# AlwinEsch/pvr.rtl.radiofm

Hardware: AMD Instinct MI355X
Metric: IQ MS/s demodulated (whole node) + achieved HBM GB/s on FIR stage (higher is better)
Workload: dtype f32

## Files before the change

pvr.rtl.radiofm_amd/csrc/fmd_batch.hip:

```cpp
#include "../../include/fmd.h"

#include <hip/hip_runtime.h>
#include <hip/hip_ext.h>

#include <algorithm>
#include <chrono>
#include <cmath>
#include <cstdio>
#include <cstdlib>
#include <cstring>
#include <deque>
#include <functional>
#include <map>
#include <memory>
#include <mutex>
#include <string>
#include <utility>
#include <vector>

#include "fmd_design.hpp"
#include "fmd_groups.hpp"
#include "fmd_kernels.hip.h"
#include "fmd_receiver.hpp"

// ... 603 lines not shown
      push(0, 0, 0);
    const size_t g = steps.size();
    for (size_t i = f; i < g; i++)
    {
      const int far = steps[std::min(i + size_t(fmd::HBF_NSET - 1), g - 1)].a_lo - steps[i].a_lo;
      if (far < 0 || far > 63 || g - i > 1023)
        return nullptr;
      steps[i].n |= unsigned(far) << fmd::HBF_FAR_SHIFT;
      if (steps[i].n & (fmd::HBF_TAIL0 | fmd::HBF_TAIL1))
        steps[i].n |= unsigned(g - i) << fmd::HBF_TAILS_SHIFT;
    }
    steps[g - 1].n |= fmd::HBF_LAST;
    fmd::HbStep hdr[2];
    static_assert(sizeof(hdr) == sizeof(tails), "HbTails in the place of two records");
    std::memcpy(hdr, &tails, sizeof(tails));
    steps.push_back(hdr[0]);
    steps.push_back(hdr[1]);
  }
  first.push_back(int(steps.size()));
  std::unique_ptr<fmd_batch::HbfPlan> pl(new fmd_batch::HbfPlan);
  pl->n_in = n_in;
  pl->S = unsigned(first.size() - 1);
  if (pl->steps.alloc(steps.size()) || pl->seg_first.alloc(first.size()) ||
      upload(pl->steps.p, steps.data(), steps.size() * sizeof(fmd::HbStep)) ||
      upload(pl->seg_first.p, first.data(), first.size() * sizeof(int)))
    return nullptr;
  if (b->hbf_plans.size() >= 16)
  {
    (void)hipDeviceSynchronize();
    b->hbf_plans.erase(b->hbf_plans.begin());
  }
  b->hbf_plans.push_back(std::move(pl));
  return b->hbf_plans.back().get();
}

bool rsr_configure(fmd_batch* b, int form)
{
  static const int forms[3][2] = {{2, 8}, {4, 4}, {2, 4}};
  const fmd::Design& d = b->des;
  const int R = forms[form][0], NW = forms[form][1];
  const double step = double(d.rs_step);
  const unsigned per_step = unsigned(NW * R);
  const unsigned span = d.rs_order + 1u + unsigned(std::ceil((per_step - 1) * step)) + 1u;
  const unsigned nbr = (span - 1u + 7u) / 8u + 2u;
  const unsigned new_rows = unsigned(std::ceil(per_step * step)) + 8u;
  b->rsr_R = 0;
  if (nbr > 39u || new_rows > unsigned(fmd::RSR_ROWS))
    return false;
  b->rsr_R = R;
  b->rsr_NW = NW;
  b->rsr_nbr = nbr;
  b->rsr_rb = int((d.rs_order + 7u) / 8u * 8u + 8u);
  const unsigned gspan = d.rs_order + 1u + unsigned(std::ceil((R - 1) * step)) + 1u;
  b->rsr_nbm = (gspan - 1u + 7u) / 8u + 2u + 1u;
  return true;
}

}

extern "C" {

const char* fmd_last_error(void)
{
  return g_err.c_str();
}

const char* fmd_version(void)
{
  return "fmd-hip 0.1 (gfx950)";
}

const char* fmd_stage_name(unsigned idx)
{
  return idx < ST_COUNT ? kStageNames[idx] : "";
}

}

namespace
{

int create_streams(fmd_batch* b)
{
  int lo = 0, hi = 0;
  HIPCHK(hipDeviceGetStreamPriorityRange(&lo, &hi));
  const int nstreams = 5;
  const int prio[5] = {hi, hi, lo, lo, lo};
  hipStream_t st4[5] = {nullptr, nullptr, nullptr, nullptr, nullptr};
  if (pick_independent_streams(nstreams, prio, st4, &b->streams_sharing) != 0)
    return fail(FMD_ERR_DEVICE, "could not create the internal streams");
  b->s_fir = st4[0];
  b->s_ser = st4[1];
  b->s_post = st4[2];
  b->s_rds = st4[3];
  b->s_lpf = st4[4];
  return FMD_OK;
}

int create_one(const fmd_params* params, unsigned n_channels, const int* tuning_shifts, int device,
               const fmd_callbacks* cb, void* user, fmd_batch* shell, fmd_batch** out)
{
  std::unique_ptr<fmd_batch> b(new fmd_batch);
  b->device = device;
  b->cparams = *params;
  b->params.sample_rate_if = params->sample_rate_if;
  b->params.tuning_offset = params->tuning_offset;
  b->params.sample_rate_pcm = params->sample_rate_pcm;
// ... 2163 lines not shown
```

pvr.rtl.radiofm_amd/csrc/fmd_k_resample.hip.h:

```cpp
#pragma once

#include "fmd_k_common.hip.h"

namespace fmd
{

__global__ void k_rs_table(const float* __restrict__ coeff, unsigned order, float p, float pstep,
                           unsigned A, float* __restrict__ ktab, unsigned row_stride, unsigned margin,
                           int* __restrict__ pidx)
{
  const unsigned i = blockIdx.x;
  if (i >= A)
    return;
  const float pf = p + (float)i * pstep;
  const int pi = (int)pf;
  const float k1 = pf - (float)pi;
  const float k0 = 1 - k1;
  for (unsigned j = threadIdx.x; j <= order; j += blockDim.x)
    ktab[(size_t)i * row_stride + margin + j] = coeff[j] * k0 + coeff[j + 1] * k1;
  if (threadIdx.x == 0)
    pidx[i] = pi;
}

#ifndef FMD_RS_R
// ... 74 lines not shown
    {
      bool fin = true;
#pragma unroll
      for (int q = 0; q < RS_B; q++)
        fin = fin && __builtin_isfinite(xs[q].x) && __builtin_isfinite(xs[q].y);
      literal = FMD_ANY_LANE(!fin);
    }
    if (!literal)
    {
#pragma unroll
      for (int q = 0; q < RS_B; q++)
      {
#pragma unroll
        for (int r = 0; r < RS_R; r++)
        {
          acc[r].x += kk[r][q] * xs[q].x;
          acc[r].y += kk[r][q] * xs[q].y;
        }
      }
    }
    else
    {
#pragma unroll
      for (int q = 0; q < RS_B; q++)
      {
#pragma unroll
        for (int r = 0; r < RS_R; r++)
        {
          const int j = t + q - off[r];
          if (j >= 0 && j <= (int)order)
          {
            acc[r].x += kk[r][q] * xs[q].x;
            acc[r].y += kk[r][q] * xs[q].y;
          }
        }
      }
    }
  }
  if (c < C)
  {
#pragma unroll
    for (int r = 0; r < RS_R; r++)
      if (r < nr)
        out[(size_t)(Hout + i0 + r) * CP + c] = make_float2(acc[r].y, acc[r].x);
  }
}


constexpr int RSR_ROWS = 96;
constexpr int RSR_HEAD = 4 + 4;

template <int R, bool FMA = false>
__device__ __forceinline__ void rs_walk_asm(fmd_f2v (&acc)[R], unsigned& off, unsigned& cnt, unsigned lane16,
                                            unsigned wrap, unsigned klo, unsigned khi, unsigned kinc);
template <>
__device__ __forceinline__ void rs_walk_asm<4, false>(fmd_f2v (&acc)[4], unsigned& off, unsigned& cnt,
                                                      unsigned lane16, unsigned wrap, unsigned klo, unsigned khi,
                                                      unsigned kinc)
{
#include "fmd_rs_walk_r4.inc"
}
template <>
__device__ __forceinline__ void rs_walk_asm<2, false>(fmd_f2v (&acc)[2], unsigned& off, unsigned& cnt,
                                                      unsigned lane16, unsigned wrap, unsigned klo, unsigned khi,
                                                      unsigned kinc)
{
#include "fmd_rs_walk_r2.inc"
}
template <>
__device__ __forceinline__ void rs_walk_asm<2, true>(fmd_f2v (&acc)[2], unsigned& off, unsigned& cnt,
                                                     unsigned lane16, unsigned wrap, unsigned klo, unsigned khi,
                                                     unsigned kinc)
{
#include "fmd_rs_walk_r2_fma.inc"
}

template <int R, int NW>
__device__ __forceinline__ void rs_warm_asm(unsigned tlo, unsigned thi, unsigned gstride, unsigned rounds,
                                            unsigned pace);
template <>
__device__ __forceinline__ void rs_warm_asm<4, 4>(unsigned tlo, unsigned thi, unsigned gstride, unsigned rounds,
                                                  unsigned pace)
{
#include "fmd_rs_warm_r4w4.inc"
}
template <>
__device__ __forceinline__ void rs_warm_asm<2, 8>(unsigned tlo, unsigned thi, unsigned gstride, unsigned rounds,
                                                  unsigned pace)
{
#include "fmd_rs_warm_r2w8.inc"
}
template <>
__device__ __forceinline__ void rs_warm_asm<2, 4>(unsigned tlo, unsigned thi, unsigned gstride, unsigned rounds,
                                                  unsigned pace)
{
#include "fmd_rs_warm_r2w4.inc"
}

template <int R, int RSR_NW>
__global__ __launch_bounds__(64) void k_rs_plan(const float* __restrict__ coeff, unsigned order, float p,
                                                float pstep, unsigned A, int RB, unsigned NBR,
                                                float* __restrict__ tab, unsigned nbm,
                                                int* __restrict__ head, int* __restrict__ steptab)
{
  const unsigned g = blockIdx.x;
  auto pidx_of = [&](unsigned i) { return (int)(p + (float)i * pstep); };
  auto extent = [&](unsigned gg, int& top, int& nb) {
    const unsigned i0 = gg * R;
    if (i0 >= A)
    {
      top = 0;
      nb = 0;
      return;
    }
    const unsigned il = min(i0 + R - 1, A - 1);
    top = (pidx_of(il) + RB) >> 3;
    const int bot = (pidx_of(i0) - (int)order + RB) >> 3;
    nb = top - bot + 1;
    nb += nb & 1;
  };
  int top, nb;
  extent(g, top, nb);
  float k0[R], k1[R];
  int pi[R];
#pragma unroll
  for (int r = 0; r < R; r++)
  {
    const unsigned i = min(g * R + r, A - 1);
    const float pf = p + (float)i * pstep;
    pi[r] = (int)pf;
    k1[r] = pf - (float)pi[r];
    k0[r] = 1 - k1[r];
  }
  for (int idx = threadIdx.x; idx < nb * 8 * R; idx += 64)
  {
    const int b = idx / (8 * R), q = (idx / R) & 7, r = idx % R;
    const int row = (top - b) * 8 + 7 - q - RB;
    float v = 0.0f;
#pragma unroll
    for (int rr = 0; rr < R; rr++)
      if (rr == r)
      {
        const int j = pi[rr] - row;
        if (j >= 0 && j <= (int)order)
          v = coeff[j] * k0[rr] + coeff[j + 1] * k1[rr];
      }
    tab[((size_t)g * nbm + b) * (8 * R) + (idx % (8 * R))] = v;
  }
  if (threadIdx.x == 0)
  {
    int* h = head + (size_t)g * RSR_HEAD;
    h[0] = top;
    h[1] = nb;
    h[2] = (int)(((unsigned)top % NBR) * 4096u);
    h[3] = 0;
#pragma unroll
    for (int r = 0; r < R; r++)
      h[4 + r] = pi[r];
    if (g % RSR_NW == 0)
    {
      int stop = 0, sbot = 0x7fffffff;
      for (unsigned w = 0; w < (unsigned)RSR_NW; w++)
      {
        int t, n;
        extent(g + w, t, n);
        if (n > 0)
        {
          stop = t;
          sbot = min(sbot, t - n + 1);
        }
      }
      steptab[2 * (g / RSR_NW)] = stop;
      steptab[2 * (g / RSR_NW) + 1] = sbot;
    }
  }
}

template <int R, int RSR_NW, bool FMA = false>
__global__ __launch_bounds__(64 * (RSR_NW + 1)) void k_resample_ring(
    const float2* __restrict__ br, unsigned Hbb, int RB, unsigned order, const float* __restrict__ tab,
    unsigned nbm, const int* __restrict__ head, const int* __restrict__ steptab, unsigned nsteps,
    unsigned steps_per_wg, unsigned NBR, unsigned A, float2* __restrict__ out, unsigned Hout, unsigned C,
    unsigned CP, unsigned prio)
{
  constexpr int RSR_PRE = RSR_ROWS / RSR_NW;
  constexpr int LEAD = 3;
  extern __shared__ __align__(16) unsigned char rsr_smem[];
  __shared__ unsigned nonfinite_s;
  const unsigned lane = threadIdx.x;
  const unsigned w = (unsigned)__builtin_amdgcn_readfirstlane((int)threadIdx.y);
  wave_prio(prio);
  const unsigned units = (CP / 64u) * nsteps;
  unsigned u0 = min(units, blockIdx.x * steps_per_wg);
  const unsigned u1 = min(units, u0 + steps_per_wg);
  if (u0 >= u1)
    return;
  unsigned c = 0, s0 = 0, s1 = 0, lane_off = 0;
  bool live = false;
  const unsigned ring_pairs = NBR * 4;
  const char* const gbase = reinterpret_cast<const char*>(br + ((ptrdiff_t)Hbb - (ptrdiff_t)RB) * (ptrdiff_t)CP);
  const size_t row_bytes = (size_t)CP * sizeof(float2);
  unsigned emax = 0u;
  auto look = [&](float2 v) {
    emax = max(emax, max(__float_as_uint(v.x) & 0x7fffffffu, __float_as_uint(v.y) & 0x7fffffffu));
  };
  auto ring_addr = [&](unsigned pair_slot, unsigned odd) {
    return reinterpret_cast<float2*>(rsr_smem + (size_t)pair_slot * 1024 + lane * 16 + odd * 8);
  };
  float2 pre[RSR_PRE];
  auto fetch = [&](int r0, int mine) {
    const char* rp = gbase + (size_t)(r0 + (int)w) * row_bytes;
#pragma unroll
    for (int n = 0; n < RSR_PRE; n++)
      if (n < mine)
      {
        const fmd_f2v v = __builtin_nontemporal_load(reinterpret_cast<const fmd_f2v*>(rp + lane_off));
        pre[n] = make_float2(v.x, v.y);
        rp += RSR_NW * row_bytes;
      }
  };
  auto stash = [&](int r0, int mine) {
    unsigned ps = ((unsigned)(r0 + (int)w) >> 1) % ring_pairs;
#pragma unroll
    for (int n = 0; n < RSR_PRE; n++)
      if (n < mine)
      {
        look(pre[n]);
        *ring_addr(ps, w & 1u) = pre[n];
        ps += RSR_NW / 2;
        ps = ps >= ring_pairs ? ps - ring_pairs : ps;
      }
    if (emax >= 0x7f800000u && live)
      nonfinite_s = 1u;
  };
  auto share = [&](int n_rows) { return (n_rows - (int)w + RSR_NW - 1) / RSR_NW; };
  const bool warmer = w == (unsigned)RSR_NW;
  auto warm = [&](unsigned step, int b0, int rounds) {
    if (rounds <= 0)
      return;
    const uint64_t ta = reinterpret_cast<uint64_t>(tab) + ((uint64_t)step * RSR_NW * nbm + (uint64_t)b0) * (32 * R);
    rs_warm_asm<R, RSR_NW>((unsigned)ta, (unsigned)(ta >> 32), nbm * (32u * R), (unsigned)rounds, 0u);
  };
  {
    const size_t gsz = (size_t)nbm * (8 * R) * sizeof(float);
    const char* t0 = reinterpret_cast<const char*>(tab);
    const size_t bytes = (size_t)nsteps * RSR_NW * gsz;
    const unsigned nx = (gridDim.x + 7u) / 8u, part = blockIdx.x / 8u;
    const size_t per = ((bytes + nx - 1) / nx + 15) & ~(size_t)15;
    const size_t lo = min(bytes, part * per), hi = min(bytes, lo + per);
    unsigned sink = 0;
    for (size_t o = lo + (size_t)(threadIdx.y * 64 + lane) * 16; o + 16 <= hi; o += (size_t)(RSR_NW + 1) * 64 * 16)
    {
      const uint4 v = *reinterpret_cast<const uint4*>(t0 + o);
      sink |= v.x ^ v.y ^ v.z ^ v.w;
    }
    if (sink == 0x7fc12345u)
      nonfinite_s = sink;
  }
  for (; u0 < u1; u0 += s1 - s0)
  {
  const unsigned grp = u0 / nsteps;
  s0 = u0 - grp * nsteps;
  s1 = min(nsteps, s0 + (u1 - u0));
  c = grp * 64 + lane;
  lane_off = c * (unsigned)sizeof(float2);
  live = c < C;
  emax = 0u;
  __syncthreads();
  if (threadIdx.x == 0 && threadIdx.y == 0)
    nonfinite_s = 0u;
  __syncthreads();
  int topb = steptab[2 * s0];
  {
    const int r_hi = topb * 8 + 7;
    for (int r0 = steptab[2 * s0 + 1] * 8; r0 <= r_hi; r0 += RSR_NW * RSR_PRE)
    {
      const int mine = warmer ? 0 : share(min(r_hi + 1 - r0, RSR_NW * RSR_PRE));
      fetch(r0, mine);
      stash(r0, mine);
    }
    if (warmer)
      warm(s0, 0, LEAD);
  }
  __syncthreads();
  for (unsigned s = s0; s < s1; s++)
  {
    const int ntop = s + 1 < s1 ? steptab[2 * (s + 1)] : topb;
    const int r_new0 = topb * 8 + 8;
    const int mine = warmer ? 0 : share((ntop - topb) * 8);
    fetch(r_new0, mine);
    if (warmer)
    {
      warm(s, LEAD, (int)nbm - 1 - LEAD);
      if (s + 1 < s1)
        warm(s + 1, 0, LEAD);
      lds_barrier();
      topb = ntop;
      lds_barrier();
      continue;
    }
    const unsigned g = s * RSR_NW + w;
    const int* __restrict__ h = head + (size_t)g * RSR_HEAD;
    const int gtop = h[0], nb = h[1];
    fmd_f2v acc[R];
#pragma unroll
    for (int r = 0; r < R; r++)
      acc[r] = fmd_f2v{0.0f, 0.0f};
    if (nb > 0)
    {
      const float* __restrict__ kp = tab + (size_t)g * nbm * (8 * R);
      if (__builtin_expect(nonfinite_s == 0u, 1))
      {
        unsigned off = (unsigned)h[2], cnt = (unsigned)nb >> 1;
        const uint64_t ka = reinterpret_cast<uint64_t>(kp);
        rs_walk_asm<R, FMA>(acc, off, cnt, (unsigned)(size_t)rsr_smem + lane * 16u, (NBR - 1u) * 4096u, (unsigned)ka,
                       (unsigned)(ka >> 32), 32u * R);
      }
      else
      {
        for (int b = 0; b < nb; b++)
        {
          const unsigned slot = (unsigned)(gtop - b) % NBR;
#pragma unroll
          for (int q = 0; q < 8; q++)
          {
            const int rowb = 7 - q;
            const float2 x = *ring_addr(slot * 4 + (unsigned)(rowb >> 1), (unsigned)rowb & 1u);
            const int row = (gtop - b) * 8 + rowb - RB;
#pragma unroll
            for (int r = 0; r < R; r++)
            {
              const int j = h[4 + r] - row;
              if (j >= 0 && j <= (int)order)
              {
                const float k = kp[(size_t)b * (8 * R) + q * R + r];
                if (FMA)
                {
                  acc[r].x = __builtin_fmaf(k, x.x, acc[r].x);
                  acc[r].y = __builtin_fmaf(k, x.y, acc[r].y);
                }
                else
                {
                  acc[r].x += k * x.x;
                  acc[r].y += k * x.y;
                }
              }
            }
          }
        }
      }
      if (live)
      {
#pragma unroll
        for (int r = 0; r < R; r++)
          if (g * R + r < A)
            out[(size_t)(Hout + g * R + r) * CP + c] = make_float2(acc[r].y, acc[r].x);
      }
    }
    lds_barrier();
    stash(r_new0, mine);
    topb = ntop;
    lds_barrier();
  }
  }
}

}
```

pvr.rtl.radiofm_amd/csrc/fmd_rs_walk_r2.inc:

```
asm volatile(
    "s_mov_b32 s34, %6\n\t"
    "s_mov_b32 s35, %7\n\t"
    "v_add_u32 v104, %2, %4\n\t"
    "s_load_dwordx16 s[36:51], s[34:35], 0x0\n\t"
    "ds_read_b128 v[76:79], v104 offset:3072\n\t"
    "ds_read_b128 v[72:75], v104 offset:2048\n\t"
    "ds_read_b128 v[68:71], v104 offset:1024\n\t"
    "ds_read_b128 v[64:67], v104\n\t"
    "s_add_u32 s34, s34, %8\n\t"
    "s_addc_u32 s35, s35, 0\n\t"
    "s_sub_u32 %2, %2, 4096\n\t"
    "s_cselect_b32 %2, %5, %2\n\t"
    "1:\n\t"
    "s_waitcnt lgkmcnt(0)\n\t"
    "v_add_u32 v104, %2, %4\n\t"
    "s_load_dwordx16 s[52:67], s[34:35], 0x0\n\t"
    "ds_read_b128 v[92:95], v104 offset:3072\n\t"
    "ds_read_b128 v[88:91], v104 offset:2048\n\t"
    "ds_read_b128 v[84:87], v104 offset:1024\n\t"
    "ds_read_b128 v[80:83], v104\n\t"
    "s_add_u32 s34, s34, %8\n\t"
    "s_addc_u32 s35, s35, 0\n\t"
    "s_sub_u32 %2, %2, 4096\n\t"
    "s_cselect_b32 %2, %5, %2\n\t"
    "v_pk_mul_f32 v[96:97], v[78:79], s[36:37] op_sel_hi:[1,0]\n\t"
    "v_pk_mul_f32 v[98:99], v[78:79], s[36:37] op_sel:[0,1]\n\t"
    "v_pk_add_f32 %0, %0, v[96:97]\n\t"
    "v_pk_mul_f32 v[100:101], v[76:77], s[38:39] op_sel_hi:[1,0]\n\t"
    "v_pk_add_f32 %1, %1, v[98:99]\n\t"
    "v_pk_mul_f32 v[102:103], v[76:77], s[38:39] op_sel:[0,1]\n\t"
    "v_pk_add_f32 %0, %0, v[100:101]\n\t"
    "v_pk_mul_f32 v[96:97], v[74:75], s[40:41] op_sel_hi:[1,0]\n\t"
    "v_pk_add_f32 %1, %1, v[102:103]\n\t"
    "v_pk_mul_f32 v[98:99], v[74:75], s[40:41] op_sel:[0,1]\n\t"
    "v_pk_add_f32 %0, %0, v[96:97]\n\t"
    "v_pk_mul_f32 v[100:101], v[72:73], s[42:43] op_sel_hi:[1,0]\n\t"
    "v_pk_add_f32 %1, %1, v[98:99]\n\t"
    "v_pk_mul_f32 v[102:103], v[72:73], s[42:43] op_sel:[0,1]\n\t"
    "v_pk_add_f32 %0, %0, v[100:101]\n\t"
    "v_pk_mul_f32 v[96:97], v[70:71], s[44:45] op_sel_hi:[1,0]\n\t"
    "v_pk_add_f32 %1, %1, v[102:103]\n\t"
    "v_pk_mul_f32 v[98:99], v[70:71], s[44:45] op_sel:[0,1]\n\t"
    "v_pk_add_f32 %0, %0, v[96:97]\n\t"
    "v_pk_mul_f32 v[100:101], v[68:69], s[46:47] op_sel_hi:[1,0]\n\t"
    "v_pk_add_f32 %1, %1, v[98:99]\n\t"
    "v_pk_mul_f32 v[102:103], v[68:69], s[46:47] op_sel:[0,1]\n\t"
    "v_pk_add_f32 %0, %0, v[100:101]\n\t"
    "v_pk_mul_f32 v[96:97], v[66:67], s[48:49] op_sel_hi:[1,0]\n\t"
    "v_pk_add_f32 %1, %1, v[102:103]\n\t"
    "v_pk_mul_f32 v[98:99], v[66:67], s[48:49] op_sel:[0,1]\n\t"
    "v_pk_add_f32 %0, %0, v[96:97]\n\t"
    "v_pk_mul_f32 v[100:101], v[64:65], s[50:51] op_sel_hi:[1,0]\n\t"
    "v_pk_add_f32 %1, %1, v[98:99]\n\t"
    "v_pk_mul_f32 v[102:103], v[64:65], s[50:51] op_sel:[0,1]\n\t"
    "v_pk_add_f32 %0, %0, v[100:101]\n\t"
    "v_pk_add_f32 %1, %1, v[102:103]\n\t"
    "s_waitcnt lgkmcnt(0)\n\t"
    "v_add_u32 v104, %2, %4\n\t"
    "s_load_dwordx16 s[36:51], s[34:35], 0x0\n\t"
    "ds_read_b128 v[76:79], v104 offset:3072\n\t"
    "ds_read_b128 v[72:75], v104 offset:2048\n\t"
    "ds_read_b128 v[68:71], v104 offset:1024\n\t"
    "ds_read_b128 v[64:67], v104\n\t"
    "s_add_u32 s34, s34, %8\n\t"
    "s_addc_u32 s35, s35, 0\n\t"
    "s_sub_u32 %2, %2, 4096\n\t"
    "s_cselect_b32 %2, %5, %2\n\t"
    "v_pk_mul_f32 v[96:97], v[94:95], s[52:53] op_sel_hi:[1,0]\n\t"
    "v_pk_mul_f32 v[98:99], v[94:95], s[52:53] op_sel:[0,1]\n\t"
    "v_pk_add_f32 %0, %0, v[96:97]\n\t"
    "v_pk_mul_f32 v[100:101], v[92:93], s[54:55] op_sel_hi:[1,0]\n\t"
    "v_pk_add_f32 %1, %1, v[98:99]\n\t"
    "v_pk_mul_f32 v[102:103], v[92:93], s[54:55] op_sel:[0,1]\n\t"
    "v_pk_add_f32 %0, %0, v[100:101]\n\t"
    "v_pk_mul_f32 v[96:97], v[90:91], s[56:57] op_sel_hi:[1,0]\n\t"
    "v_pk_add_f32 %1, %1, v[102:103]\n\t"
    "v_pk_mul_f32 v[98:99], v[90:91], s[56:57] op_sel:[0,1]\n\t"
    "v_pk_add_f32 %0, %0, v[96:97]\n\t"
    "v_pk_mul_f32 v[100:101], v[88:89], s[58:59] op_sel_hi:[1,0]\n\t"
    "v_pk_add_f32 %1, %1, v[98:99]\n\t"
    "v_pk_mul_f32 v[102:103], v[88:89], s[58:59] op_sel:[0,1]\n\t"
    "v_pk_add_f32 %0, %0, v[100:101]\n\t"
    "v_pk_mul_f32 v[96:97], v[86:87], s[60:61] op_sel_hi:[1,0]\n\t"
    "v_pk_add_f32 %1, %1, v[102:103]\n\t"
    "v_pk_mul_f32 v[98:99], v[86:87], s[60:61] op_sel:[0,1]\n\t"
    "v_pk_add_f32 %0, %0, v[96:97]\n\t"
    "v_pk_mul_f32 v[100:101], v[84:85], s[62:63] op_sel_hi:[1,0]\n\t"
    "v_pk_add_f32 %1, %1, v[98:99]\n\t"
    "v_pk_mul_f32 v[102:103], v[84:85], s[62:63] op_sel:[0,1]\n\t"
    "v_pk_add_f32 %0, %0, v[100:101]\n\t"
    "v_pk_mul_f32 v[96:97], v[82:83], s[64:65] op_sel_hi:[1,0]\n\t"
    "v_pk_add_f32 %1, %1, v[102:103]\n\t"
    "v_pk_mul_f32 v[98:99], v[82:83], s[64:65] op_sel:[0,1]\n\t"
    "v_pk_add_f32 %0, %0, v[96:97]\n\t"
    "v_pk_mul_f32 v[100:101], v[80:81], s[66:67] op_sel_hi:[1,0]\n\t"
    "v_pk_add_f32 %1, %1, v[98:99]\n\t"
    "v_pk_mul_f32 v[102:103], v[80:81], s[66:67] op_sel:[0,1]\n\t"
    "v_pk_add_f32 %0, %0, v[100:101]\n\t"
    "v_pk_add_f32 %1, %1, v[102:103]\n\t"
    "s_sub_u32 %3, %3, 1\n\t"
    "s_cmp_lg_u32 %3, 0\n\t"
    "s_cbranch_scc1 1b\n\t"
    "s_waitcnt lgkmcnt(0)\n\t"
    : "+v"(acc[0]), "+v"(acc[1]), "+s"(off), "+s"(cnt)
    : "v"(lane16), "s"(wrap), "s"(klo), "s"(khi), "s"(kinc)
    : "v64", "v65", "v66", "v67", "v68", "v69", "v70", "v71", "v72", "v73", "v74", "v75", "v76",
      "v77", "v78", "v79", "v80", "v81", "v82", "v83", "v84", "v85", "v86", "v87", "v88", "v89",
      "v90", "v91", "v92", "v93", "v94", "v95", "v96", "v97", "v98", "v99", "v100", "v101", "v102",
      "v103", "v104", "s34", "s35", "s36", "s37", "s38", "s39", "s40", "s41", "s42", "s43", "s44",
      "s45", "s46", "s47", "s48", "s49", "s50", "s51", "s52", "s53", "s54", "s55", "s56", "s57",
      "s58", "s59", "s60", "s61", "s62", "s63", "s64", "s65", "s66", "s67", "scc", "memory");
```

pvr.rtl.radiofm_amd/csrc/fmd_rs_walk_r2_fma.inc:

```
asm volatile(
    "s_mov_b32 s34, %6\n\t"
    "s_mov_b32 s35, %7\n\t"
    "v_add_u32 v104, %2, %4\n\t"
    "s_load_dwordx16 s[36:51], s[34:35], 0x0\n\t"
    "ds_read_b128 v[76:79], v104 offset:3072\n\t"
    "ds_read_b128 v[72:75], v104 offset:2048\n\t"
    "ds_read_b128 v[68:71], v104 offset:1024\n\t"
    "ds_read_b128 v[64:67], v104\n\t"
    "s_add_u32 s34, s34, %8\n\t"
    "s_addc_u32 s35, s35, 0\n\t"
    "s_sub_u32 %2, %2, 4096\n\t"
    "s_cselect_b32 %2, %5, %2\n\t"
    "1:\n\t"
    "s_waitcnt lgkmcnt(0)\n\t"
    "v_add_u32 v104, %2, %4\n\t"
    "s_load_dwordx16 s[52:67], s[34:35], 0x0\n\t"
    "ds_read_b128 v[92:95], v104 offset:3072\n\t"
    "ds_read_b128 v[88:91], v104 offset:2048\n\t"
    "ds_read_b128 v[84:87], v104 offset:1024\n\t"
    "ds_read_b128 v[80:83], v104\n\t"
    "s_add_u32 s34, s34, %8\n\t"
    "s_addc_u32 s35, s35, 0\n\t"
    "s_sub_u32 %2, %2, 4096\n\t"
    "s_cselect_b32 %2, %5, %2\n\t"
    "v_pk_fma_f32 %0, v[78:79], s[36:37], %0 op_sel_hi:[1,0,1]\n\t"
    "v_pk_fma_f32 %1, v[78:79], s[36:37], %1 op_sel:[0,1,0]\n\t"
    "v_pk_fma_f32 %0, v[76:77], s[38:39], %0 op_sel_hi:[1,0,1]\n\t"
    "v_pk_fma_f32 %1, v[76:77], s[38:39], %1 op_sel:[0,1,0]\n\t"
    "v_pk_fma_f32 %0, v[74:75], s[40:41], %0 op_sel_hi:[1,0,1]\n\t"
    "v_pk_fma_f32 %1, v[74:75], s[40:41], %1 op_sel:[0,1,0]\n\t"
    "v_pk_fma_f32 %0, v[72:73], s[42:43], %0 op_sel_hi:[1,0,1]\n\t"
    "v_pk_fma_f32 %1, v[72:73], s[42:43], %1 op_sel:[0,1,0]\n\t"
    "v_pk_fma_f32 %0, v[70:71], s[44:45], %0 op_sel_hi:[1,0,1]\n\t"
    "v_pk_fma_f32 %1, v[70:71], s[44:45], %1 op_sel:[0,1,0]\n\t"
    "v_pk_fma_f32 %0, v[68:69], s[46:47], %0 op_sel_hi:[1,0,1]\n\t"
    "v_pk_fma_f32 %1, v[68:69], s[46:47], %1 op_sel:[0,1,0]\n\t"
    "v_pk_fma_f32 %0, v[66:67], s[48:49], %0 op_sel_hi:[1,0,1]\n\t"
    "v_pk_fma_f32 %1, v[66:67], s[48:49], %1 op_sel:[0,1,0]\n\t"
    "v_pk_fma_f32 %0, v[64:65], s[50:51], %0 op_sel_hi:[1,0,1]\n\t"
    "v_pk_fma_f32 %1, v[64:65], s[50:51], %1 op_sel:[0,1,0]\n\t"
    "s_waitcnt lgkmcnt(0)\n\t"
    "v_add_u32 v104, %2, %4\n\t"
    "s_load_dwordx16 s[36:51], s[34:35], 0x0\n\t"
    "ds_read_b128 v[76:79], v104 offset:3072\n\t"
    "ds_read_b128 v[72:75], v104 offset:2048\n\t"
    "ds_read_b128 v[68:71], v104 offset:1024\n\t"
    "ds_read_b128 v[64:67], v104\n\t"
    "s_add_u32 s34, s34, %8\n\t"
    "s_addc_u32 s35, s35, 0\n\t"
    "s_sub_u32 %2, %2, 4096\n\t"
    "s_cselect_b32 %2, %5, %2\n\t"
    "v_pk_fma_f32 %0, v[94:95], s[52:53], %0 op_sel_hi:[1,0,1]\n\t"
    "v_pk_fma_f32 %1, v[94:95], s[52:53], %1 op_sel:[0,1,0]\n\t"
    "v_pk_fma_f32 %0, v[92:93], s[54:55], %0 op_sel_hi:[1,0,1]\n\t"
    "v_pk_fma_f32 %1, v[92:93], s[54:55], %1 op_sel:[0,1,0]\n\t"
    "v_pk_fma_f32 %0, v[90:91], s[56:57], %0 op_sel_hi:[1,0,1]\n\t"
    "v_pk_fma_f32 %1, v[90:91], s[56:57], %1 op_sel:[0,1,0]\n\t"
    "v_pk_fma_f32 %0, v[88:89], s[58:59], %0 op_sel_hi:[1,0,1]\n\t"
    "v_pk_fma_f32 %1, v[88:89], s[58:59], %1 op_sel:[0,1,0]\n\t"
    "v_pk_fma_f32 %0, v[86:87], s[60:61], %0 op_sel_hi:[1,0,1]\n\t"
    "v_pk_fma_f32 %1, v[86:87], s[60:61], %1 op_sel:[0,1,0]\n\t"
    "v_pk_fma_f32 %0, v[84:85], s[62:63], %0 op_sel_hi:[1,0,1]\n\t"
    "v_pk_fma_f32 %1, v[84:85], s[62:63], %1 op_sel:[0,1,0]\n\t"
    "v_pk_fma_f32 %0, v[82:83], s[64:65], %0 op_sel_hi:[1,0,1]\n\t"
    "v_pk_fma_f32 %1, v[82:83], s[64:65], %1 op_sel:[0,1,0]\n\t"
    "v_pk_fma_f32 %0, v[80:81], s[66:67], %0 op_sel_hi:[1,0,1]\n\t"
    "v_pk_fma_f32 %1, v[80:81], s[66:67], %1 op_sel:[0,1,0]\n\t"
    "s_sub_u32 %3, %3, 1\n\t"
    "s_cmp_lg_u32 %3, 0\n\t"
    "s_cbranch_scc1 1b\n\t"
    "s_waitcnt lgkmcnt(0)\n\t"
    : "+v"(acc[0]), "+v"(acc[1]), "+s"(off), "+s"(cnt)
    : "v"(lane16), "s"(wrap), "s"(klo), "s"(khi), "s"(kinc)
    : "v64", "v65", "v66", "v67", "v68", "v69", "v70", "v71", "v72", "v73", "v74", "v75", "v76",
      "v77", "v78", "v79", "v80", "v81", "v82", "v83", "v84", "v85", "v86", "v87", "v88", "v89",
      "v90", "v91", "v92", "v93", "v94", "v95", "v96", "v97", "v98", "v99", "v100", "v101", "v102",
      "v103", "v104", "s34", "s35", "s36", "s37", "s38", "s39", "s40", "s41", "s42", "s43", "s44",
      "s45", "s46", "s47", "s48", "s49", "s50", "s51", "s52", "s53", "s54", "s55", "s56", "s57",
      "s58", "s59", "s60", "s61", "s62", "s63", "s64", "s65", "s66", "s67", "scc", "memory");
```

pvr.rtl.radiofm_amd/csrc/fmd_rs_walk_r4.inc:

```
asm volatile(
    "s_mov_b32 s34, %8\n\t"
    "s_mov_b32 s35, %9\n\t"
    "v_add_u32 v104, %4, %6\n\t"
    "s_load_dwordx16 s[36:51], s[34:35], 0x0\n\t"
    "s_load_dwordx16 s[52:67], s[34:35], 0x40\n\t"
    "ds_read_b128 v[76:79], v104 offset:3072\n\t"
    "ds_read_b128 v[72:75], v104 offset:2048\n\t"
    "ds_read_b128 v[68:71], v104 offset:1024\n\t"
    "ds_read_b128 v[64:67], v104\n\t"
    "s_add_u32 s34, s34, %10\n\t"
    "s_addc_u32 s35, s35, 0\n\t"
    "s_sub_u32 %4, %4, 4096\n\t"
    "s_cselect_b32 %4, %7, %4\n\t"
    "1:\n\t"
    "s_waitcnt lgkmcnt(0)\n\t"
    "v_add_u32 v104, %4, %6\n\t"
    "s_load_dwordx16 s[68:83], s[34:35], 0x0\n\t"
    "s_load_dwordx16 s[84:99], s[34:35], 0x40\n\t"
    "ds_read_b128 v[92:95], v104 offset:3072\n\t"
    "ds_read_b128 v[88:91], v104 offset:2048\n\t"
    "ds_read_b128 v[84:87], v104 offset:1024\n\t"
    "ds_read_b128 v[80:83], v104\n\t"
    "s_add_u32 s34, s34, %10\n\t"
    "s_addc_u32 s35, s35, 0\n\t"
    "s_sub_u32 %4, %4, 4096\n\t"
    "s_cselect_b32 %4, %7, %4\n\t"
    "v_pk_mul_f32 v[96:97], v[78:79], s[36:37] op_sel_hi:[1,0]\n\t"
    "v_pk_mul_f32 v[98:99], v[78:79], s[36:37] op_sel:[0,1]\n\t"
    "v_pk_add_f32 %0, %0, v[96:97]\n\t"
    "v_pk_mul_f32 v[100:101], v[78:79], s[38:39] op_sel_hi:[1,0]\n\t"
    "v_pk_add_f32 %1, %1, v[98:99]\n\t"
    "v_pk_mul_f32 v[102:103], v[78:79], s[38:39] op_sel:[0,1]\n\t"
    "v_pk_add_f32 %2, %2, v[100:101]\n\t"
    "v_pk_mul_f32 v[96:97], v[76:77], s[40:41] op_sel_hi:[1,0]\n\t"
    "v_pk_add_f32 %3, %3, v[102:103]\n\t"
    "v_pk_mul_f32 v[98:99], v[76:77], s[40:41] op_sel:[0,1]\n\t"
    "v_pk_add_f32 %0, %0, v[96:97]\n\t"
    "v_pk_mul_f32 v[100:101], v[76:77], s[42:43] op_sel_hi:[1,0]\n\t"
    "v_pk_add_f32 %1, %1, v[98:99]\n\t"
    "v_pk_mul_f32 v[102:103], v[76:77], s[42:43] op_sel:[0,1]\n\t"
    "v_pk_add_f32 %2, %2, v[100:101]\n\t"
    "v_pk_mul_f32 v[96:97], v[74:75], s[44:45] op_sel_hi:[1,0]\n\t"
    "v_pk_add_f32 %3, %3, v[102:103]\n\t"
    "v_pk_mul_f32 v[98:99], v[74:75], s[44:45] op_sel:[0,1]\n\t"
    "v_pk_add_f32 %0, %0, v[96:97]\n\t"
    "v_pk_mul_f32 v[100:101], v[74:75], s[46:47] op_sel_hi:[1,0]\n\t"
    "v_pk_add_f32 %1, %1, v[98:99]\n\t"
    "v_pk_mul_f32 v[102:103], v[74:75], s[46:47] op_sel:[0,1]\n\t"
    "v_pk_add_f32 %2, %2, v[100:101]\n\t"
    "v_pk_mul_f32 v[96:97], v[72:73], s[48:49] op_sel_hi:[1,0]\n\t"
    "v_pk_add_f32 %3, %3, v[102:103]\n\t"
    "v_pk_mul_f32 v[98:99], v[72:73], s[48:49] op_sel:[0,1]\n\t"
    "v_pk_add_f32 %0, %0, v[96:97]\n\t"
    "v_pk_mul_f32 v[100:101], v[72:73], s[50:51] op_sel_hi:[1,0]\n\t"
    "v_pk_add_f32 %1, %1, v[98:99]\n\t"
    "v_pk_mul_f32 v[102:103], v[72:73], s[50:51] op_sel:[0,1]\n\t"
    "v_pk_add_f32 %2, %2, v[100:101]\n\t"
    "v_pk_mul_f32 v[96:97], v[70:71], s[52:53] op_sel_hi:[1,0]\n\t"
    "v_pk_add_f32 %3, %3, v[102:103]\n\t"
    "v_pk_mul_f32 v[98:99], v[70:71], s[52:53] op_sel:[0,1]\n\t"
    "v_pk_add_f32 %0, %0, v[96:97]\n\t"
    "v_pk_mul_f32 v[100:101], v[70:71], s[54:55] op_sel_hi:[1,0]\n\t"
    "v_pk_add_f32 %1, %1, v[98:99]\n\t"
    "v_pk_mul_f32 v[102:103], v[70:71], s[54:55] op_sel:[0,1]\n\t"
    "v_pk_add_f32 %2, %2, v[100:101]\n\t"
    "v_pk_mul_f32 v[96:97], v[68:69], s[56:57] op_sel_hi:[1,0]\n\t"
// ... 50 lines not shown
    "v_pk_add_f32 %2, %2, v[100:101]\n\t"
    "v_pk_mul_f32 v[96:97], v[90:91], s[76:77] op_sel_hi:[1,0]\n\t"
    "v_pk_add_f32 %3, %3, v[102:103]\n\t"
    "v_pk_mul_f32 v[98:99], v[90:91], s[76:77] op_sel:[0,1]\n\t"
    "v_pk_add_f32 %0, %0, v[96:97]\n\t"
    "v_pk_mul_f32 v[100:101], v[90:91], s[78:79] op_sel_hi:[1,0]\n\t"
    "v_pk_add_f32 %1, %1, v[98:99]\n\t"
    "v_pk_mul_f32 v[102:103], v[90:91], s[78:79] op_sel:[0,1]\n\t"
    "v_pk_add_f32 %2, %2, v[100:101]\n\t"
    "v_pk_mul_f32 v[96:97], v[88:89], s[80:81] op_sel_hi:[1,0]\n\t"
    "v_pk_add_f32 %3, %3, v[102:103]\n\t"
    "v_pk_mul_f32 v[98:99], v[88:89], s[80:81] op_sel:[0,1]\n\t"
    "v_pk_add_f32 %0, %0, v[96:97]\n\t"
    "v_pk_mul_f32 v[100:101], v[88:89], s[82:83] op_sel_hi:[1,0]\n\t"
    "v_pk_add_f32 %1, %1, v[98:99]\n\t"
    "v_pk_mul_f32 v[102:103], v[88:89], s[82:83] op_sel:[0,1]\n\t"
    "v_pk_add_f32 %2, %2, v[100:101]\n\t"
    "v_pk_mul_f32 v[96:97], v[86:87], s[84:85] op_sel_hi:[1,0]\n\t"
    "v_pk_add_f32 %3, %3, v[102:103]\n\t"
    "v_pk_mul_f32 v[98:99], v[86:87], s[84:85] op_sel:[0,1]\n\t"
    "v_pk_add_f32 %0, %0, v[96:97]\n\t"
    "v_pk_mul_f32 v[100:101], v[86:87], s[86:87] op_sel_hi:[1,0]\n\t"
    "v_pk_add_f32 %1, %1, v[98:99]\n\t"
    "v_pk_mul_f32 v[102:103], v[86:87], s[86:87] op_sel:[0,1]\n\t"
    "v_pk_add_f32 %2, %2, v[100:101]\n\t"
    "v_pk_mul_f32 v[96:97], v[84:85], s[88:89] op_sel_hi:[1,0]\n\t"
    "v_pk_add_f32 %3, %3, v[102:103]\n\t"
    "v_pk_mul_f32 v[98:99], v[84:85], s[88:89] op_sel:[0,1]\n\t"
    "v_pk_add_f32 %0, %0, v[96:97]\n\t"
    "v_pk_mul_f32 v[100:101], v[84:85], s[90:91] op_sel_hi:[1,0]\n\t"
    "v_pk_add_f32 %1, %1, v[98:99]\n\t"
    "v_pk_mul_f32 v[102:103], v[84:85], s[90:91] op_sel:[0,1]\n\t"
    "v_pk_add_f32 %2, %2, v[100:101]\n\t"
    "v_pk_mul_f32 v[96:97], v[82:83], s[92:93] op_sel_hi:[1,0]\n\t"
    "v_pk_add_f32 %3, %3, v[102:103]\n\t"
    "v_pk_mul_f32 v[98:99], v[82:83], s[92:93] op_sel:[0,1]\n\t"
    "v_pk_add_f32 %0, %0, v[96:97]\n\t"
    "v_pk_mul_f32 v[100:101], v[82:83], s[94:95] op_sel_hi:[1,0]\n\t"
    "v_pk_add_f32 %1, %1, v[98:99]\n\t"
    "v_pk_mul_f32 v[102:103], v[82:83], s[94:95] op_sel:[0,1]\n\t"
    "v_pk_add_f32 %2, %2, v[100:101]\n\t"
    "v_pk_mul_f32 v[96:97], v[80:81], s[96:97] op_sel_hi:[1,0]\n\t"
    "v_pk_add_f32 %3, %3, v[102:103]\n\t"
    "v_pk_mul_f32 v[98:99], v[80:81], s[96:97] op_sel:[0,1]\n\t"
    "v_pk_add_f32 %0, %0, v[96:97]\n\t"
    "v_pk_mul_f32 v[100:101], v[80:81], s[98:99] op_sel_hi:[1,0]\n\t"
    "v_pk_add_f32 %1, %1, v[98:99]\n\t"
    "v_pk_mul_f32 v[102:103], v[80:81], s[98:99] op_sel:[0,1]\n\t"
    "v_pk_add_f32 %2, %2, v[100:101]\n\t"
    "v_pk_add_f32 %3, %3, v[102:103]\n\t"
    "s_sub_u32 %5, %5, 1\n\t"
    "s_cmp_lg_u32 %5, 0\n\t"
    "s_cbranch_scc1 1b\n\t"
    "s_waitcnt lgkmcnt(0)\n\t"
    : "+v"(acc[0]), "+v"(acc[1]), "+v"(acc[2]), "+v"(acc[3]), "+s"(off), "+s"(cnt)
    : "v"(lane16), "s"(wrap), "s"(klo), "s"(khi), "s"(kinc)
    : "v64", "v65", "v66", "v67", "v68", "v69", "v70", "v71", "v72", "v73", "v74", "v75", "v76",
      "v77", "v78", "v79", "v80", "v81", "v82", "v83", "v84", "v85", "v86", "v87", "v88", "v89",
      "v90", "v91", "v92", "v93", "v94", "v95", "v96", "v97", "v98", "v99", "v100", "v101", "v102",
      "v103", "v104", "s34", "s35", "s36", "s37", "s38", "s39", "s40", "s41", "s42", "s43", "s44",
      "s45", "s46", "s47", "s48", "s49", "s50", "s51", "s52", "s53", "s54", "s55", "s56", "s57",
      "s58", "s59", "s60", "s61", "s62", "s63", "s64", "s65", "s66", "s67", "s68", "s69", "s70",
      "s71", "s72", "s73", "s74", "s75", "s76", "s77", "s78", "s79", "s80", "s81", "s82", "s83",
      "s84", "s85", "s86", "s87", "s88", "s89", "s90", "s91", "s92", "s93", "s94", "s95", "s96",
      "s97", "s98", "s99", "scc", "memory");
```

Before: 295,800.

## Drop even-block padding in resample walk, add odd tail, prefetch group headers

Stops rounding each group's coefficient block count up to an even number and adds an odd-tail path to the asm walk loops, so zero-padded blocks are no longer multiplied. The per-group header now carries the next step's top, and the kernel loads headers as int4 records one step ahead, replacing the separate steptab and header reads. The non-finite check is moved out of stash so it overlaps the compute. This adds branches to the hand-written asm and changes table sizing, which may be fragile.

```diff
diff --git a/pvr.rtl.radiofm_amd/csrc/fmd_batch.hip b/pvr.rtl.radiofm_amd/csrc/fmd_batch.hip
--- a/pvr.rtl.radiofm_amd/csrc/fmd_batch.hip
+++ b/pvr.rtl.radiofm_amd/csrc/fmd_batch.hip
@@ -679,7 +679,7 @@
   b->rsr_nbr = nbr;
   b->rsr_rb = int((d.rs_order + 7u) / 8u * 8u + 8u);
   const unsigned gspan = d.rs_order + 1u + unsigned(std::ceil((R - 1) * step)) + 1u;
-  b->rsr_nbm = (gspan - 1u + 7u) / 8u + 2u + 1u;
+  b->rsr_nbm = (gspan - 1u + 7u) / 8u + 1u + 1u;
   return true;
 }
 
diff --git a/pvr.rtl.radiofm_amd/csrc/fmd_k_resample.hip.h b/pvr.rtl.radiofm_amd/csrc/fmd_k_resample.hip.h
--- a/pvr.rtl.radiofm_amd/csrc/fmd_k_resample.hip.h
+++ b/pvr.rtl.radiofm_amd/csrc/fmd_k_resample.hip.h
@@ -150,25 +150,25 @@
 
 template <int R, bool FMA = false>
 __device__ __forceinline__ void rs_walk_asm(fmd_f2v (&acc)[R], unsigned& off, unsigned& cnt, unsigned lane16,
-                                            unsigned wrap, unsigned klo, unsigned khi, unsigned kinc);
+                                            unsigned wrap, unsigned klo, unsigned khi, unsigned kinc, unsigned odd);
 template <>
 __device__ __forceinline__ void rs_walk_asm<4, false>(fmd_f2v (&acc)[4], unsigned& off, unsigned& cnt,
                                                       unsigned lane16, unsigned wrap, unsigned klo, unsigned khi,
-                                                      unsigned kinc)
+                                                      unsigned kinc, unsigned odd)
 {
 #include "fmd_rs_walk_r4.inc"
 }
 template <>
 __device__ __forceinline__ void rs_walk_asm<2, false>(fmd_f2v (&acc)[2], unsigned& off, unsigned& cnt,
                                                       unsigned lane16, unsigned wrap, unsigned klo, unsigned khi,
-                                                      unsigned kinc)
+                                                      unsigned kinc, unsigned odd)
 {
 #include "fmd_rs_walk_r2.inc"
 }
 template <>
 __device__ __forceinline__ void rs_walk_asm<2, true>(fmd_f2v (&acc)[2], unsigned& off, unsigned& cnt,
                                                      unsigned lane16, unsigned wrap, unsigned klo, unsigned khi,
-                                                     unsigned kinc)
+                                                     unsigned kinc, unsigned odd)
 {
 #include "fmd_rs_walk_r2_fma.inc"
 }
@@ -215,7 +215,20 @@
     top = (pidx_of(il) + RB) >> 3;
     const int bot = (pidx_of(i0) - (int)order + RB) >> 3;
     nb = top - bot + 1;
-    nb += nb & 1;
+  };
+  auto step_extent = [&](unsigned s, int& stop, int& sbot) {
+    stop = 0;
+    sbot = 0x7fffffff;
+    for (unsigned w = 0; w < (unsigned)RSR_NW; w++)
+    {
+      int t, n;
+      extent(s * RSR_NW + w, t, n);
+      if (n > 0)
+      {
+        stop = t;
+        sbot = min(sbot, t - n + 1);
+      }
+    }
   };
   int top, nb;
   extent(g, top, nb);
@@ -248,28 +261,21 @@
   if (threadIdx.x == 0)
   {
     int* h = head + (size_t)g * RSR_HEAD;
+    const unsigned s = g / RSR_NW;
+    int stop, sbot, ntop, nbot;
+    step_extent(s, stop, sbot);
+    step_extent(s + 1, ntop, nbot);
     h[0] = top;
     h[1] = nb;
     h[2] = (int)(((unsigned)top % NBR) * 4096u);
-    h[3] = 0;
+    h[3] = (s + 1) * RSR_NW * R < A ? ntop : stop;
 #pragma unroll
     for (int r = 0; r < R; r++)
       h[4 + r] = pi[r];
     if (g % RSR_NW == 0)
     {
-      int stop = 0, sbot = 0x7fffffff;
-      for (unsigned w = 0; w < (unsigned)RSR_NW; w++)
-      {
-        int t, n;
-        extent(g + w, t, n);
-        if (n > 0)
-        {
-          stop = t;
-          sbot = min(sbot, t - n + 1);
-        }
-      }
-      steptab[2 * (g / RSR_NW)] = stop;
-      steptab[2 * (g / RSR_NW) + 1] = sbot;
+      steptab[2 * s] = stop;
+      steptab[2 * s + 1] = sbot;
     }
   }
 }
@@ -317,19 +323,24 @@
         rp += RSR_NW * row_bytes;
       }
   };
+  auto inspect = [&](int mine) {
+#pragma unroll
+    for (int n = 0; n < RSR_PRE; n++)
+      if (n < mine)
+        look(pre[n]);
+    if (emax >= 0x7f800000u && live)
+      nonfinite_s = 1u;
+  };
   auto stash = [&](int r0, int mine) {
     unsigned ps = ((unsigned)(r0 + (int)w) >> 1) % ring_pairs;
 #pragma unroll
     for (int n = 0; n < RSR_PRE; n++)
       if (n < mine)
       {
-        look(pre[n]);
         *ring_addr(ps, w & 1u) = pre[n];
         ps += RSR_NW / 2;
         ps = ps >= ring_pairs ? ps - ring_pairs : ps;
       }
-    if (emax >= 0x7f800000u && live)
-      nonfinite_s = 1u;
   };
   auto share = [&](int n_rows) { return (n_rows - (int)w + RSR_NW - 1) / RSR_NW; };
   const bool warmer = w == (unsigned)RSR_NW;
@@ -375,15 +386,21 @@
     {
       const int mine = warmer ? 0 : share(min(r_hi + 1 - r0, RSR_NW * RSR_PRE));
       fetch(r0, mine);
+      inspect(mine);
       stash(r0, mine);
     }
     if (warmer)
       warm(s0, 0, LEAD);
   }
+  const int4* __restrict__ recs = reinterpret_cast<const int4*>(head);
+  static_assert(RSR_HEAD == 8, "two int4 per group");
+  int4 cur = recs[2 * (s0 * RSR_NW + (warmer ? 0u : w))];
   __syncthreads();
   for (unsigned s = s0; s < s1; s++)
   {
-    const int ntop = s + 1 < s1 ? steptab[2 * (s + 1)] : topb;
+    const int4 st = cur;
+    unsigned flag = nonfinite_s;
+    const int ntop = s + 1 < s1 ? st.w : topb;
     const int r_new0 = topb * 8 + 8;
     const int mine = warmer ? 0 : share((ntop - topb) * 8);
     fetch(r_new0, mine);
@@ -399,7 +416,9 @@
     }
     const unsigned g = s * RSR_NW + w;
     const int* __restrict__ h = head + (size_t)g * RSR_HEAD;
-    const int gtop = h[0], nb = h[1];
+    const int gtop = st.x, nb = st.y;
+    asm volatile("" : "+v"(flag)::"memory");
+    cur = recs[2 * ((s + 1 < s1 ? s + 1 : s) * RSR_NW + w)];
     fmd_f2v acc[R];
 #pragma unroll
     for (int r = 0; r < R; r++)
@@ -407,12 +426,12 @@
     if (nb > 0)
     {
       const float* __restrict__ kp = tab + (size_t)g * nbm * (8 * R);
-      if (__builtin_expect(nonfinite_s == 0u, 1))
-      {
-        unsigned off = (unsigned)h[2], cnt = (unsigned)nb >> 1;
+      if (__builtin_expect(flag == 0u, 1))
+      {
+        unsigned off = (unsigned)st.z, cnt = (unsigned)nb >> 1;
         const uint64_t ka = reinterpret_cast<uint64_t>(kp);
         rs_walk_asm<R, FMA>(acc, off, cnt, (unsigned)(size_t)rsr_smem + lane * 16u, (NBR - 1u) * 4096u, (unsigned)ka,
-                       (unsigned)(ka >> 32), 32u * R);
+                       (unsigned)(ka >> 32), 32u * R, (unsigned)nb & 1u);
       }
       else
       {
@@ -447,13 +466,15 @@
           }
         }
       }
-      if (live)
-      {
-#pragma unroll
-        for (int r = 0; r < R; r++)
-          if (g * R + r < A)
-            out[(size_t)(Hout + g * R + r) * CP + c] = make_float2(acc[r].y, acc[r].x);
-      }
+    }
+    inspect(mine);
+    asm volatile("" : "+v"(emax)::"memory");
+    if (nb > 0 && live)
+    {
+#pragma unroll
+      for (int r = 0; r < R; r++)
+        if (g * R + r < A)
+          out[(size_t)(Hout + g * R + r) * CP + c] = make_float2(acc[r].y, acc[r].x);
     }
     lds_barrier();
     stash(r_new0, mine);
diff --git a/pvr.rtl.radiofm_amd/csrc/fmd_rs_walk_r2.inc b/pvr.rtl.radiofm_amd/csrc/fmd_rs_walk_r2.inc
--- a/pvr.rtl.radiofm_amd/csrc/fmd_rs_walk_r2.inc
+++ b/pvr.rtl.radiofm_amd/csrc/fmd_rs_walk_r2.inc
@@ -11,6 +11,8 @@
     "s_addc_u32 s35, s35, 0\n\t"
     "s_sub_u32 %2, %2, 4096\n\t"
     "s_cselect_b32 %2, %5, %2\n\t"
+    "s_cmp_eq_u32 %3, 0\n\t"
+    "s_cbranch_scc1 2f\n\t"
     "1:\n\t"
     "s_waitcnt lgkmcnt(0)\n\t"
     "v_add_u32 v104, %2, %4\n\t"
@@ -101,9 +103,45 @@
     "s_sub_u32 %3, %3, 1\n\t"
     "s_cmp_lg_u32 %3, 0\n\t"
     "s_cbranch_scc1 1b\n\t"
+    "2:\n\t"
     "s_waitcnt lgkmcnt(0)\n\t"
+    "s_cmp_eq_u32 %9, 0\n\t"
+    "s_cbranch_scc1 3f\n\t"
+    "v_pk_mul_f32 v[96:97], v[78:79], s[36:37] op_sel_hi:[1,0]\n\t"
+    "v_pk_mul_f32 v[98:99], v[78:79], s[36:37] op_sel:[0,1]\n\t"
+    "v_pk_add_f32 %0, %0, v[96:97]\n\t"
+    "v_pk_mul_f32 v[100:101], v[76:77], s[38:39] op_sel_hi:[1,0]\n\t"
+    "v_pk_add_f32 %1, %1, v[98:99]\n\t"
+    "v_pk_mul_f32 v[102:103], v[76:77], s[38:39] op_sel:[0,1]\n\t"
+    "v_pk_add_f32 %0, %0, v[100:101]\n\t"
+    "v_pk_mul_f32 v[96:97], v[74:75], s[40:41] op_sel_hi:[1,0]\n\t"
+    "v_pk_add_f32 %1, %1, v[102:103]\n\t"
+    "v_pk_mul_f32 v[98:99], v[74:75], s[40:41] op_sel:[0,1]\n\t"
+    "v_pk_add_f32 %0, %0, v[96:97]\n\t"
+    "v_pk_mul_f32 v[100:101], v[72:73], s[42:43] op_sel_hi:[1,0]\n\t"
+    "v_pk_add_f32 %1, %1, v[98:99]\n\t"
+    "v_pk_mul_f32 v[102:103], v[72:73], s[42:43] op_sel:[0,1]\n\t"
+    "v_pk_add_f32 %0, %0, v[100:101]\n\t"
+    "v_pk_mul_f32 v[96:97], v[70:71], s[44:45] op_sel_hi:[1,0]\n\t"
+    "v_pk_add_f32 %1, %1, v[102:103]\n\t"
+    "v_pk_mul_f32 v[98:99], v[70:71], s[44:45] op_sel:[0,1]\n\t"
+    "v_pk_add_f32 %0, %0, v[96:97]\n\t"
+    "v_pk_mul_f32 v[100:101], v[68:69], s[46:47] op_sel_hi:[1,0]\n\t"
+    "v_pk_add_f32 %1, %1, v[98:99]\n\t"
+    "v_pk_mul_f32 v[102:103], v[68:69], s[46:47] op_sel:[0,1]\n\t"
+    "v_pk_add_f32 %0, %0, v[100:101]\n\t"
+    "v_pk_mul_f32 v[96:97], v[66:67], s[48:49] op_sel_hi:[1,0]\n\t"
+    "v_pk_add_f32 %1, %1, v[102:103]\n\t"
+    "v_pk_mul_f32 v[98:99], v[66:67], s[48:49] op_sel:[0,1]\n\t"
+    "v_pk_add_f32 %0, %0, v[96:97]\n\t"
+    "v_pk_mul_f32 v[100:101], v[64:65], s[50:51] op_sel_hi:[1,0]\n\t"
+    "v_pk_add_f32 %1, %1, v[98:99]\n\t"
+    "v_pk_mul_f32 v[102:103], v[64:65], s[50:51] op_sel:[0,1]\n\t"
+    "v_pk_add_f32 %0, %0, v[100:101]\n\t"
+    "v_pk_add_f32 %1, %1, v[102:103]\n\t"
+    "3:\n\t"
     : "+v"(acc[0]), "+v"(acc[1]), "+s"(off), "+s"(cnt)
-    : "v"(lane16), "s"(wrap), "s"(klo), "s"(khi), "s"(kinc)
+    : "v"(lane16), "s"(wrap), "s"(klo), "s"(khi), "s"(kinc), "s"(odd)
     : "v64", "v65", "v66", "v67", "v68", "v69", "v70", "v71", "v72", "v73", "v74", "v75", "v76",
       "v77", "v78", "v79", "v80", "v81", "v82", "v83", "v84", "v85", "v86", "v87", "v88", "v89",
       "v90", "v91", "v92", "v93", "v94", "v95", "v96", "v97", "v98", "v99", "v100", "v101", "v102",
diff --git a/pvr.rtl.radiofm_amd/csrc/fmd_rs_walk_r2_fma.inc b/pvr.rtl.radiofm_amd/csrc/fmd_rs_walk_r2_fma.inc
--- a/pvr.rtl.radiofm_amd/csrc/fmd_rs_walk_r2_fma.inc
+++ b/pvr.rtl.radiofm_amd/csrc/fmd_rs_walk_r2_fma.inc
@@ -11,6 +11,8 @@
     "s_addc_u32 s35, s35, 0\n\t"
     "s_sub_u32 %2, %2, 4096\n\t"
     "s_cselect_b32 %2, %5, %2\n\t"
+    "s_cmp_eq_u32 %3, 0\n\t"
+    "s_cbranch_scc1 2f\n\t"
     "1:\n\t"
     "s_waitcnt lgkmcnt(0)\n\t"
     "v_add_u32 v104, %2, %4\n\t"
@@ -69,9 +71,29 @@
     "s_sub_u32 %3, %3, 1\n\t"
     "s_cmp_lg_u32 %3, 0\n\t"
     "s_cbranch_scc1 1b\n\t"
+    "2:\n\t"
     "s_waitcnt lgkmcnt(0)\n\t"
+    "s_cmp_eq_u32 %9, 0\n\t"
+    "s_cbranch_scc1 3f\n\t"
+    "v_pk_fma_f32 %0, v[78:79], s[36:37], %0 op_sel_hi:[1,0,1]\n\t"
+    "v_pk_fma_f32 %1, v[78:79], s[36:37], %1 op_sel:[0,1,0]\n\t"
+    "v_pk_fma_f32 %0, v[76:77], s[38:39], %0 op_sel_hi:[1,0,1]\n\t"
+    "v_pk_fma_f32 %1, v[76:77], s[38:39], %1 op_sel:[0,1,0]\n\t"
+    "v_pk_fma_f32 %0, v[74:75], s[40:41], %0 op_sel_hi:[1,0,1]\n\t"
+    "v_pk_fma_f32 %1, v[74:75], s[40:41], %1 op_sel:[0,1,0]\n\t"
+    "v_pk_fma_f32 %0, v[72:73], s[42:43], %0 op_sel_hi:[1,0,1]\n\t"
+    "v_pk_fma_f32 %1, v[72:73], s[42:43], %1 op_sel:[0,1,0]\n\t"
+    "v_pk_fma_f32 %0, v[70:71], s[44:45], %0 op_sel_hi:[1,0,1]\n\t"
+    "v_pk_fma_f32 %1, v[70:71], s[44:45], %1 op_sel:[0,1,0]\n\t"
+    "v_pk_fma_f32 %0, v[68:69], s[46:47], %0 op_sel_hi:[1,0,1]\n\t"
+    "v_pk_fma_f32 %1, v[68:69], s[46:47], %1 op_sel:[0,1,0]\n\t"
+    "v_pk_fma_f32 %0, v[66:67], s[48:49], %0 op_sel_hi:[1,0,1]\n\t"
+    "v_pk_fma_f32 %1, v[66:67], s[48:49], %1 op_sel:[0,1,0]\n\t"
+    "v_pk_fma_f32 %0, v[64:65], s[50:51], %0 op_sel_hi:[1,0,1]\n\t"
+    "v_pk_fma_f32 %1, v[64:65], s[50:51], %1 op_sel:[0,1,0]\n\t"
+    "3:\n\t"
     : "+v"(acc[0]), "+v"(acc[1]), "+s"(off), "+s"(cnt)
-    : "v"(lane16), "s"(wrap), "s"(klo), "s"(khi), "s"(kinc)
+    : "v"(lane16), "s"(wrap), "s"(klo), "s"(khi), "s"(kinc), "s"(odd)
     : "v64", "v65", "v66", "v67", "v68", "v69", "v70", "v71", "v72", "v73", "v74", "v75", "v76",
       "v77", "v78", "v79", "v80", "v81", "v82", "v83", "v84", "v85", "v86", "v87", "v88", "v89",
       "v90", "v91", "v92", "v93", "v94", "v95", "v96", "v97", "v98", "v99", "v100", "v101", "v102",
diff --git a/pvr.rtl.radiofm_amd/csrc/fmd_rs_walk_r4.inc b/pvr.rtl.radiofm_amd/csrc/fmd_rs_walk_r4.inc
--- a/pvr.rtl.radiofm_amd/csrc/fmd_rs_walk_r4.inc
+++ b/pvr.rtl.radiofm_amd/csrc/fmd_rs_walk_r4.inc
@@ -12,6 +12,8 @@
     "s_addc_u32 s35, s35, 0\n\t"
     "s_sub_u32 %4, %4, 4096\n\t"
     "s_cselect_b32 %4, %7, %4\n\t"
+    "s_cmp_eq_u32 %5, 0\n\t"
+    "s_cbranch_scc1 2f\n\t"
     "1:\n\t"
     "s_waitcnt lgkmcnt(0)\n\t"
     "v_add_u32 v104, %4, %6\n\t"
@@ -168,9 +170,77 @@
     "s_sub_u32 %5, %5, 1\n\t"
     "s_cmp_lg_u32 %5, 0\n\t"
     "s_cbranch_scc1 1b\n\t"
+    "2:\n\t"
     "s_waitcnt lgkmcnt(0)\n\t"
+    "s_cmp_eq_u32 %11, 0\n\t"
+    "s_cbranch_scc1 3f\n\t"
+    "v_pk_mul_f32 v[96:97], v[78:79], s[36:37] op_sel_hi:[1,0]\n\t"
+    "v_pk_mul_f32 v[98:99], v[78:79], s[36:37] op_sel:[0,1]\n\t"
+    "v_pk_add_f32 %0, %0, v[96:97]\n\t"
+    "v_pk_mul_f32 v[100:101], v[78:79], s[38:39] op_sel_hi:[1,0]\n\t"
+    "v_pk_add_f32 %1, %1, v[98:99]\n\t"
+    "v_pk_mul_f32 v[102:103], v[78:79], s[38:39] op_sel:[0,1]\n\t"
+    "v_pk_add_f32 %2, %2, v[100:101]\n\t"
+    "v_pk_mul_f32 v[96:97], v[76:77], s[40:41] op_sel_hi:[1,0]\n\t"
+    "v_pk_add_f32 %3, %3, v[102:103]\n\t"
+    "v_pk_mul_f32 v[98:99], v[76:77], s[40:41] op_sel:[0,1]\n\t"
+    "v_pk_add_f32 %0, %0, v[96:97]\n\t"
+    "v_pk_mul_f32 v[100:101], v[76:77], s[42:43] op_sel_hi:[1,0]\n\t"
+    "v_pk_add_f32 %1, %1, v[98:99]\n\t"
+    "v_pk_mul_f32 v[102:103], v[76:77], s[42:43] op_sel:[0,1]\n\t"
+    "v_pk_add_f32 %2, %2, v[100:101]\n\t"
+    "v_pk_mul_f32 v[96:97], v[74:75], s[44:45] op_sel_hi:[1,0]\n\t"
+    "v_pk_add_f32 %3, %3, v[102:103]\n\t"
+    "v_pk_mul_f32 v[98:99], v[74:75], s[44:45] op_sel:[0,1]\n\t"
+    "v_pk_add_f32 %0, %0, v[96:97]\n\t"
+    "v_pk_mul_f32 v[100:101], v[74:75], s[46:47] op_sel_hi:[1,0]\n\t"
+    "v_pk_add_f32 %1, %1, v[98:99]\n\t"
+    "v_pk_mul_f32 v[102:103], v[74:75], s[46:47] op_sel:[0,1]\n\t"
+    "v_pk_add_f32 %2, %2, v[100:101]\n\t"
+    "v_pk_mul_f32 v[96:97], v[72:73], s[48:49] op_sel_hi:[1,0]\n\t"
+    "v_pk_add_f32 %3, %3, v[102:103]\n\t"
+    "v_pk_mul_f32 v[98:99], v[72:73], s[48:49] op_sel:[0,1]\n\t"
+    "v_pk_add_f32 %0, %0, v[96:97]\n\t"
+    "v_pk_mul_f32 v[100:101], v[72:73], s[50:51] op_sel_hi:[1,0]\n\t"
+    "v_pk_add_f32 %1, %1, v[98:99]\n\t"
+    "v_pk_mul_f32 v[102:103], v[72:73], s[50:51] op_sel:[0,1]\n\t"
+    "v_pk_add_f32 %2, %2, v[100:101]\n\t"
+    "v_pk_mul_f32 v[96:97], v[70:71], s[52:53] op_sel_hi:[1,0]\n\t"
+    "v_pk_add_f32 %3, %3, v[102:103]\n\t"
+    "v_pk_mul_f32 v[98:99], v[70:71], s[52:53] op_sel:[0,1]\n\t"
+    "v_pk_add_f32 %0, %0, v[96:97]\n\t"
+    "v_pk_mul_f32 v[100:101], v[70:71], s[54:55] op_sel_hi:[1,0]\n\t"
+    "v_pk_add_f32 %1, %1, v[98:99]\n\t"
+    "v_pk_mul_f32 v[102:103], v[70:71], s[54:55] op_sel:[0,1]\n\t"
+    "v_pk_add_f32 %2, %2, v[100:101]\n\t"
+    "v_pk_mul_f32 v[96:97], v[68:69], s[56:57] op_sel_hi:[1,0]\n\t"
+    "v_pk_add_f32 %3, %3, v[102:103]\n\t"
+    "v_pk_mul_f32 v[98:99], v[68:69], s[56:57] op_sel:[0,1]\n\t"
+    "v_pk_add_f32 %0, %0, v[96:97]\n\t"
+    "v_pk_mul_f32 v[100:101], v[68:69], s[58:59] op_sel_hi:[1,0]\n\t"
+    "v_pk_add_f32 %1, %1, v[98:99]\n\t"
+    "v_pk_mul_f32 v[102:103], v[68:69], s[58:59] op_sel:[0,1]\n\t"
+    "v_pk_add_f32 %2, %2, v[100:101]\n\t"
+    "v_pk_mul_f32 v[96:97], v[66:67], s[60:61] op_sel_hi:[1,0]\n\t"
+    "v_pk_add_f32 %3, %3, v[102:103]\n\t"
+    "v_pk_mul_f32 v[98:99], v[66:67], s[60:61] op_sel:[0,1]\n\t"
+    "v_pk_add_f32 %0, %0, v[96:97]\n\t"
+    "v_pk_mul_f32 v[100:101], v[66:67], s[62:63] op_sel_hi:[1,0]\n\t"
+    "v_pk_add_f32 %1, %1, v[98:99]\n\t"
+    "v_pk_mul_f32 v[102:103], v[66:67], s[62:63] op_sel:[0,1]\n\t"
+    "v_pk_add_f32 %2, %2, v[100:101]\n\t"
+    "v_pk_mul_f32 v[96:97], v[64:65], s[64:65] op_sel_hi:[1,0]\n\t"
+    "v_pk_add_f32 %3, %3, v[102:103]\n\t"
+    "v_pk_mul_f32 v[98:99], v[64:65], s[64:65] op_sel:[0,1]\n\t"
+    "v_pk_add_f32 %0, %0, v[96:97]\n\t"
+    "v_pk_mul_f32 v[100:101], v[64:65], s[66:67] op_sel_hi:[1,0]\n\t"
+    "v_pk_add_f32 %1, %1, v[98:99]\n\t"
+    "v_pk_mul_f32 v[102:103], v[64:65], s[66:67] op_sel:[0,1]\n\t"
+    "v_pk_add_f32 %2, %2, v[100:101]\n\t"
+    "v_pk_add_f32 %3, %3, v[102:103]\n\t"
+    "3:\n\t"
     : "+v"(acc[0]), "+v"(acc[1]), "+v"(acc[2]), "+v"(acc[3]), "+s"(off), "+s"(cnt)
-    : "v"(lane16), "s"(wrap), "s"(klo), "s"(khi), "s"(kinc)
+    : "v"(lane16), "s"(wrap), "s"(klo), "s"(khi), "s"(kinc), "s"(odd)
     : "v64", "v65", "v66", "v67", "v68", "v69", "v70", "v71", "v72", "v73", "v74", "v75", "v76",
       "v77", "v78", "v79", "v80", "v81", "v82", "v83", "v84", "v85", "v86", "v87", "v88", "v89",
       "v90", "v91", "v92", "v93", "v94", "v95", "v96", "v97", "v98", "v99", "v100", "v101", "v102",
```

Result: no change. 297,900, median of 6 (+0.7%).
